# guy3540/Acoustic_Locating_VQ-VAE

Hardware: AMD Instinct MI355X
Metric: spectrograms/sec (train step), speech VQ-VAE default config (higher is better)
Workload: dtype x3mx_hb

## Files before the change

acoustic_locating_vq-vae_amd/csrc/alvq_common.h:

```cpp
#pragma once
#include <hip/hip_runtime.h>
#include <stdint.h>
#include <stdio.h>

#include "../../include/alvq.h"

namespace alvq {

void set_error(const char* fmt, ...);

enum Option { OPT_WIDE_MIN_TILES, OPT_FX_ROWS, OPT_FX_NARROW, OPT_FX_EPI, OPT_CONV_V2, OPT_CONV_K3, OPT_WGRAD_V3, OPT_VQ_REG, OPT_PHAT_LDS, OPT_COUNT };
long option(int id);

inline int check_launch(const char* what) {
  hipError_t e = hipGetLastError();
  if (e != hipSuccess) {
    set_error("%s: %s", what, hipGetErrorString(e));
    return (int)e;
  }
  return ALVQ_OK;
}

#define ALVQ_REQUIRE(cond, code, ...)  \
  do {                                 \
    if (!(cond)) {                     \
      alvq::set_error(__VA_ARGS__);    \
      return (code);                   \
    }                                  \
  } while (0)

struct DeviceOnce {
  bool done[64] = {};
  bool need() {
    int d = 0;
    if (hipGetDevice(&d) != hipSuccess || d < 0 || d >= 64) return true;
    if (done[d]) return false;
    done[d] = true;
    return true;
  }
};

constexpr int kWave = 64;
constexpr int kNumXcd = 8;

// ... 19 lines not shown
```

acoustic_locating_vq-vae_amd/csrc/api.hip:

```cpp
#include <stdarg.h>
#include <stdlib.h>
#include <string.h>

#include <atomic>

#include "alvq_common.h"

namespace alvq {
static thread_local char g_err[512] = "";
void set_error(const char* fmt, ...) {
  va_list ap;
  va_start(ap, fmt);
  vsnprintf(g_err, sizeof(g_err), fmt, ap);
  va_end(ap);
}

struct OptionSpec { const char* name; const char* env; long def; };
static const OptionSpec kSpecs[OPT_COUNT] = {
    {"wide_min_tiles", "ALVQ_WIDE_MIN_TILES", 192},
    {"fx_rows", "ALVQ_FX_ROWS", 0},
    {"fx_narrow", "ALVQ_FX_NARROW", 1},
    {"fx_epi", "ALVQ_FX_EPI", 1},
    {"conv_v2", "ALVQ_CONV_V2", 1},
    {"conv_k3", "ALVQ_CONV_K3", 1},
    {"wgrad_v3", "ALVQ_WGRAD_V3", 3},
    {"vq_reg", "ALVQ_VQ_REG", 1},
    {"phat_lds", "ALVQ_PHAT_LDS", 1},
};
static std::atomic<long> g_opt[OPT_COUNT];
static std::atomic<int> g_opt_ready{0};
static void options_init() {
  if (g_opt_ready.load(std::memory_order_acquire)) return;
  for (int i = 0; i < OPT_COUNT; ++i) {
    const char* e = getenv(kSpecs[i].env);
    g_opt[i].store(e ? atol(e) : kSpecs[i].def, std::memory_order_relaxed);
  }
  g_opt_ready.store(1, std::memory_order_release);
}
long option(int id) {
  options_init();
  return g_opt[id].load(std::memory_order_relaxed);
}
}

extern "C" const char* alvq_version(void) { return "alvq 0.4.0 (gfx950)"; }
extern "C" const char* alvq_last_error(void) { return alvq::g_err; }

extern "C" int alvq_set_option(const char* name, int64_t value) {
  ALVQ_REQUIRE(name, ALVQ_EINVAL, "alvq_set_option: null name");
  alvq::options_init();
  for (int i = 0; i < alvq::OPT_COUNT; ++i)
    if (!strcmp(name, alvq::kSpecs[i].name)) {
      alvq::g_opt[i].store((long)value, std::memory_order_relaxed);
      return ALVQ_OK;
    }
// ... 14 lines not shown
```

acoustic_locating_vq-vae_amd/csrc/conv1d_bf16.hip:

```cpp
#include <stdlib.h>

#include "alvq_common.h"
#include "bf16_common.h"
#include "conv_tile.h"
#include "nlc_host.h"

namespace alvq {

template <int KW, int OUT, int F16 = 0>
__global__ __launch_bounds__(256, 2) void conv1d_bf16_kernel(ConvBArgs a) {
  constexpr int PAD = (KW - 1) / 2;
  extern __shared__ __attribute__((aligned(16))) unsigned char lds[];
  unsigned char* const Xb = lds;
  unsigned char* const Wb = lds + 2 * XBYTES;

  const int tid = threadIdx.x, lane = tid & 63;
  const int wave = __builtin_amdgcn_readfirstlane(tid >> 6);
  const int li = lane & 15, kq = lane >> 4;
  const int wm0 = (wave >> 1) * 64, wn0 = (wave & 1) * 64;

  const ConvTileOrigin o = conv_tile_origin<TB_M, TB_R>(a);
  const int m0 = o.m0, r0 = o.r0;
  const int Cp = a.Cp;

// ... 45 lines not shown
    }
    const unsigned char* Wc = Wb + (step & 1) * WBYTES;
    const unsigned char* Xc = Xb + (chunk & 1) * XBYTES;
#pragma unroll
    for (int s = 0; s < 2; ++s) {
      bf16x8_t af[4], bfr[4];
#pragma unroll
      for (int mi = 0; mi < 4; ++mi) {
        const int row = wm0 + mi * 16 + li;
        af[mi] = *(const bf16x8_t*)(Wc + row * 128 + (((s * 4 + kq) ^ (row & 7)) << 4));
      }
#pragma unroll
      for (int ni = 0; ni < 4; ++ni) {
        const int row = wn0 + ni * 16 + li + tap;
        bfr[ni] = *(const bf16x8_t*)(Xc + row * 128 + (((s * 4 + kq) ^ (row & 7)) << 4));
      }
#pragma unroll
      for (int mi = 0; mi < 4; ++mi)
#pragma unroll
        for (int ni = 0; ni < 4; ++ni)
          acc[mi][ni] = elem_mfma16<F16>(af[mi], bfr[ni], acc[mi][ni]);
    }
    asm volatile("s_waitcnt vmcnt(0)" ::: "memory");
    __syncthreads();
    tap = ntap;
    chunk = nchunk;
  }

  if (OUT == 0) {
    wave_epilogue_bf16<4, 4, F16>(a, acc, m0, r0, li, kq, wm0, wn0);
    return;
  }
  const float oscale = a.out_scale ? *a.out_scale : 1.f;
  float* Cs = (float*)lds;
#pragma unroll
  for (int mi = 0; mi < 4; ++mi)
#pragma unroll
    for (int ni = 0; ni < 4; ++ni) {
      const int rl = wn0 + ni * 16 + li, ml = wm0 + mi * 16 + kq * 4;
      *(f32x4*)(Cs + rl * CS + ml) = acc[mi][ni];
    }
  __syncthreads();

  const int Lp1 = a.L + 1, ndata = a.B * Lp1;
  {
    const int rl = tid & 127, row = r0 + rl;
    int b, l;
    const bool ok = row_valid(row, Lp1, ndata, &b, &l);
    if (ok) {
      for (int ml = tid >> 7; ml < TB_M; ml += 2) {
        const int m = m0 + ml;
        if (m >= a.M) break;
        a.y_ncl[((long)b * a.M + m) * a.L + l] = (Cs[rl * CS + ml] + (a.bias ? a.bias[m] : 0.f)) * oscale;
      }
    }
  }
}

template <int F16 = 0>
__global__ __launch_bounds__(256) void ncl_to_nlc_kernel(const float* x, u16* y, int B, int C, int L, int Cp, int rows_total,
                                                         const float* scale = nullptr) {
  __shared__ float tile[32][33];
  elem_saturate<F16>();
  const float sc = scale ? *scale : 1.f;
  const int ct = Cp / 32, rt = (rows_total + 31) / 32;
  const int r0 = (blockIdx.x / ct) * 32, c0 = (blockIdx.x % ct) * 32;
  (void)rt;
  const int tx = threadIdx.x & 31, ty = threadIdx.x >> 5;
  const int Lp1 = L + 1, ndata = B * Lp1;
#pragma unroll
  for (int i = 0; i < 4; ++i) {
    const int c = c0 + ty + 8 * i, row = r0 + tx;
    int b, l;
    const bool ok = row_valid(row, Lp1, ndata, &b, &l) && c < C;
    tile[ty + 8 * i][tx] = ok ? x[((long)b * C + c) * L + l] * sc : 0.f;
  }
  __syncthreads();
#pragma unroll
  for (int i = 0; i < 4; ++i) {
    const int row = r0 + ty + 8 * i, c = c0 + tx;
    if (row < rows_total) y[(long)row * Cp + c] = F16 ? (u16)(elem_pk<1>(tile[tx][ty + 8 * i], 0.f) & 0xffffu) : f2bf(tile[tx][ty + 8 * i]);
  }
}

template <int F16 = 0>
__global__ __launch_bounds__(256) void nlc_to_ncl_kernel(const u16* x, float* y, int B, int C, int L, int Cp, int rows_total,
                                                         const float* scale = nullptr) {
  __shared__ float tile[32][33];
  const float sc = scale ? *scale : 1.f;
// ... 190 lines not shown
```

acoustic_locating_vq-vae_amd/csrc/conv1d_bf16x3.hip:

```cpp
#include <stdlib.h>

#include "alvq_common.h"
#include "bf16_common.h"
#include "conv_tile.h"
#include "nlc_host.h"
#include "wgrad_bias_reduce.h"
#include "wgrad_reduce.h"
#include "wgrad_tile.h"

namespace alvq {

struct ConvX3Args {
  ConvBArgs b;
  long x_plane, wp_plane, y_plane;
};

__device__ __forceinline__ void split2(float v, u16& hi, u16& lo) {
  hi = f2bf(v);
  lo = f2bf(v - bf2f(hi));
}

__device__ __forceinline__ void split_pack8(const float (&v)[8], u32x4& hi, u32x4& lo) {
#pragma unroll
  for (int e = 0; e < 4; ++e) {
    hi[e] = f2bf_pk(v[2 * e], v[2 * e + 1]);
    lo[e] = f2bf_pk(v[2 * e] - __uint_as_float(hi[e] << 16), v[2 * e + 1] - __uint_as_float(hi[e] & 0xffff0000u));
  }
}

template <int NNI>
__device__ __forceinline__ void wave_epilogue_x3(const ConvX3Args& ax, const f32x4 (&acc)[8][NNI], int m0, int r0, int li,
                                                 int kq, int wm0, int wn0) {
  const ConvBArgs& a = ax.b;
  const int Lp1 = a.L + 1, ndata = a.B * Lp1;
  const int mb0 = m0 + wm0 + (kq & 1) * 16 + (kq >> 1) * 8;
  const long pl = ax.y_plane;
#pragma unroll
  for (int ni = 0; ni < NNI; ++ni) {
    const int row = r0 + wn0 + ni * 16 + li;
    int b, l;
    const bool ok = row_valid(row, Lp1, ndata, &b, &l);
    const bool gaps = !__all(ok);
    const long o0 = (long)row * a.Mop + mb0;
    u16x8 s1h[4], s1l[4], mk[4];
#pragma unroll
    for (int mp = 0; mp < 8; mp += 2) {
      if (m0 + wm0 + mp * 16 >= a.Mop) continue;
// ... 55 lines not shown
          hi[e] = ok ? hi[e] : 0u;
          lo[e] = ok ? lo[e] : 0u;
        }
      }
      *(u32x4*)(a.y + o) = hi;
      *(u32x4*)(a.y + pl + o) = lo;
      if (a.y2) {
        const u16x8 ph = *(const u16x8*)(a.post + o), pq = *(const u16x8*)(a.post + pl + o);
#pragma unroll
        for (int e = 0; e < 8; ++e) v[e] += bf2f(ph[e]) + bf2f(pq[e]);
        split_pack8(v, hi, lo);
        if (gaps) {
#pragma unroll
          for (int e = 0; e < 4; ++e) {
            hi[e] = ok ? hi[e] : 0u;
            lo[e] = ok ? lo[e] : 0u;
          }
        }
        *(u32x4*)(a.y2 + o) = hi;
        *(u32x4*)(a.y2 + pl + o) = lo;
      }
    }
  }
}

template <int NNI, int OPS>
__device__ __forceinline__ void wave_epilogue_x3_ordered(const ConvX3Args& ax, f32x4 (&acc)[8][NNI], int m0, int r0, int li,
                                                         int kq, int wm0, int wn0) {
  const ConvBArgs& a = ax.b;
  const int Lp1 = a.L + 1, ndata = a.B * Lp1;
  const int mb0 = m0 + wm0 + (kq & 1) * 16 + (kq >> 1) * 8;
  const long pl = ax.y_plane;
  const long o00 = (long)(r0 + wn0 + li) * a.Mop + mb0, oblk = (long)16 * a.Mop;
  u16x8 s1h[4], s1l[4];
  auto request = [&](int ni) {
#pragma unroll
    for (int p = 0; p < 4; ++p) {
      s1h[p] = *(const u16x8*)(a.skip1 + o00 + ni * oblk + p * 32);
      s1l[p] = *(const u16x8*)(a.skip1 + pl + o00 + ni * oblk + p * 32);
    }
  };
  if (OPS == 1) request(0);
  if (OPS == 2) {
#pragma unroll
    for (int mi = 0; mi < 8; ++mi) {
      const int c0 = m0 + wm0 + mi * 16 + kq * 4;
      f32x4 bv;
      if (m0 + wm0 + (mi & ~1) * 16 + 32 <= a.M) {
        bv = *(const f32x4*)(a.bias + c0);
      } else {
#pragma unroll
        for (int e = 0; e < 4; ++e) bv[e] = (c0 + e < a.M) ? a.bias[c0 + e] : 0.f;
      }
#pragma unroll
      for (int ni = 0; ni < NNI; ++ni)
#pragma unroll
        for (int e = 0; e < 4; ++e) acc[mi][ni][e] += bv[e];
    }
  }
  __builtin_amdgcn_sched_barrier(0);
#pragma unroll
  for (int ni = 0; ni < NNI; ++ni) {
    int b, l;
    const bool ok = row_valid(r0 + wn0 + ni * 16 + li, Lp1, ndata, &b, &l);
    const bool gaps = !__all(ok);
    u32x4 hi[4], lo[4];
#pragma unroll
    for (int p = 0; p < 4; ++p) {
      float v[8];
#pragma unroll
      for (int e = 0; e < 4; ++e) {
        const u32x2 r = __builtin_amdgcn_permlane16_swap(__float_as_uint(acc[2 * p][ni][e]), __float_as_uint(acc[2 * p + 1][ni][e]),
                                                         false, false);
        v[e] = __uint_as_float(r[0]);
        v[e + 4] = __uint_as_float(r[1]);
      }
      if (OPS == 1) {
#pragma unroll
        for (int e = 0; e < 8; ++e) v[e] += bf2f(s1h[p][e]) + bf2f(s1l[p][e]);
      }
      if (a.relu & 1) {
#pragma unroll
        for (int e = 0; e < 8; ++e) v[e] = fmaxf(v[e], 0.f);
      }
      split_pack8(v, hi[p], lo[p]);
      if (gaps) {
#pragma unroll
        for (int e = 0; e < 4; ++e) {
          hi[p][e] = ok ? hi[p][e] : 0u;
          lo[p][e] = ok ? lo[p][e] : 0u;
        }
      }
    }
    __builtin_amdgcn_sched_barrier(0);
    if (OPS == 1 && ni + 1 < NNI) request(ni + 1);
    __builtin_amdgcn_sched_barrier(0);
#pragma unroll
    for (int p = 0; p < 4; ++p) {
      *(u32x4*)(a.y + o00 + ni * oblk + p * 32) = hi[p];
      *(u32x4*)(a.y + pl + o00 + ni * oblk + p * 32) = lo[p];
    }
  }
}


template <int OUT, int KW, int NNI = 4>
__global__ __launch_bounds__(512, 2) void conv1d_bf16x3_kernel(ConvX3Args ax) {
  static_assert(NNI == 4 || NNI == 2 || NNI == 1, "4, 2 or 1 row fragments per wave");
  typedef ConvRings G;
  constexpr int MT = NNI == 4 ? G::M : 128;
  constexpr int RT = NNI == 1 ? 128 : G::R;
  const ConvBArgs& a = ax.b;
  extern __shared__ __attribute__((aligned(16))) unsigned char lds[];
  const int tid = threadIdx.x, lane = tid & 63;
  const int wave = __builtin_amdgcn_readfirstlane(tid >> 6);
  const int li = lane & 15, kq = lane >> 4;
  const int wm0 = NNI == 4 ? (wave >> 2) * 128 : 0, wn0 = NNI == 4 ? (wave & 3) * 64 : wave * 16 * NNI;

  const ConvTileOrigin o = conv_tile_origin<MT, RT>(a);
  const int m0 = o.m0, r0 = o.r0;
  const int Cp = a.Cp;
  const int srow = slab64_lane(lane).row;
  const unsigned lane_off = slab64_lane_off(lane, Cp);
  const long tap_w = (long)a.Mp128 * Cp * 2;
  const long row16 = (long)Cp * 32;
  const long wpl = ax.wp_plane * 2, xpl = ax.x_plane * 2;
  const char* const wb = (const char*)(a.wp + ((long)m0 + wave * 32) * Cp);
  const char* const xb = (const char*)(a.x + ((long)r0 - (KW - 1) / 2 + wave * 32) * Cp);
  const ConvRingStager<KW, MT, RT, false> st(wave, srow, lane_off, tap_w, row16, wpl, xpl, wb, xb);

  const int loffA = slab64_frag16(li, kq, 0);
  int loffB[KW];
#pragma unroll
// ... 38 lines not shown
  X3_MM(fa0, BY, 0) X3_SB X3_RDA(fa1, 1, WS, 1) X3_SB                                              \
  X3_MM(fa0, BY, 1) X3_SB                                                                          \
  asm volatile("s_waitcnt vmcnt(0) lgkmcnt(0)" ::: "memory");                                      \
  __builtin_amdgcn_s_barrier();                                                                    \
  if (early) { DMA_ }                                                                              \
  X3_MM(fa1, BX, 0) X3_SB X3_RDA(fa0, 0, NWS, 0) X3_RDB(BY, NXS, NTAP, 0) X3_SB                    \
  if (!early) { DMA_ }                                                                             \
  X3_MM(fa1, BX, 1) X3_SB X3_RDA(fa0, 1, NWS, 0) X3_SB

  if (KW == 3) {
    for (int c = 0; c < nch; c += 2) {
      const int t = 3 * c;
      X3_TILE(0, 0, 0, 1, 0, 1, fb0, fb1, if (t + 2 < n) st.issueW(lds, t + 2); if (c + 1 < nch) st.issueX(lds, c + 1, 0);)
      X3_TILE(1, 0, 1, 0, 0, 2, fb1, fb0, if (t + 3 < n) st.issueW(lds, t + 3); if (c + 1 < nch) st.issueX(lds, c + 1, 1);)
      X3_TILE(0, 0, 2, 1, 1, 0, fb0, fb1, if (t + 4 < n) st.issueW(lds, t + 4);)
      X3_TILE(1, 1, 0, 0, 1, 1, fb1, fb0, if (t + 5 < n) st.issueW(lds, t + 5); if (c + 2 < nch) st.issueX(lds, c + 2, 0);)
      X3_TILE(0, 1, 1, 1, 1, 2, fb0, fb1, if (t + 6 < n) st.issueW(lds, t + 6); if (c + 2 < nch) st.issueX(lds, c + 2, 1);)
      X3_TILE(1, 1, 2, 0, 0, 0, fb1, fb0, if (t + 7 < n) st.issueW(lds, t + 7);)
    }
  } else {
    for (int t = 0; t < n; t += 2) {
      X3_TILE(0, 0, 0, 1, 1, 0, fb0, fb1, if (t + 2 < n) { st.issueW(lds, t + 2); st.issueX(lds, t + 2, 0); st.issueX(lds, t + 2, 1); })
      X3_TILE(1, 1, 0, 0, 0, 0, fb1, fb0, if (t + 3 < n) { st.issueW(lds, t + 3); st.issueX(lds, t + 3, 0); st.issueX(lds, t + 3, 1); })
    }
  }
#undef X3_TILE
#undef X3_SB
#undef X3_MM
#undef X3_RDB
#undef X3_RDA
  asm volatile("s_nop 15\n\ts_nop 15" ::: "memory");

  if constexpr (OUT == 0) {
    const bool plain = !a.skip2 && !a.mask && !a.y2 && m0 + wm0 + 128 <= a.Mop;
    if (plain && a.skip1 && !a.bias) wave_epilogue_x3_ordered<NNI, 1>(ax, acc, m0, r0, li, kq, wm0, wn0);
    else if (plain && a.bias && !a.skip1) wave_epilogue_x3_ordered<NNI, 2>(ax, acc, m0, r0, li, kq, wm0, wn0);
    else wave_epilogue_x3(ax, acc, m0, r0, li, kq, wm0, wn0);
    return;
  }
  __syncthreads();
  conv_store_ncl<false, MT, RT>(a, lds, m0, r0, tid, nullptr, [&](float* Cs, int slab) {
    if ((wn0 >> 6) == slab) store_frags16<C_SLAB_STRIDE>(Cs, acc, li, kq, wm0, wn0 & 63);
  });
}

struct WgradX3Args {
  const u16* dy[WGRAD_MAXSEG];
  const u16* x[WGRAD_MAXSEG];
  int nseg;
  float* partial;
  float* bias_partial;
  long dy_plane, x_plane;
  int Mp, Cp, M, C;
  int mtiles, ctiles, splits, chunks_per_split, total_rows;
};

template <int KW, int NCF>
__global__ __launch_bounds__(512, 2) void conv1d_wgrad_bf16x3_kernel(WgradX3Args a) {
  constexpr int MT = 128, CT = 4 * NCF * 16;
  typedef WgradSlabs<KW, MT, CT, 2> Slabs;
  constexpr int YRB = Slabs::YRB, XRB = Slabs::XRB, YBYTES = Slabs::YBYTES, XBYTES = Slabs::XBYTES;
  extern __shared__ __attribute__((aligned(16))) unsigned char lds[];

  const int tid = threadIdx.x, lane = tid & 63;
  const int wave = __builtin_amdgcn_readfirstlane(tid >> 6);
  const int wm0 = (wave >> 2) * 64, wc0 = (wave & 3) * NCF * 16;
  const WgradWork w = wgrad_work<MT, CT>(a);
  const int n = w.n;
  WgradStager<WgradX3Args, KW, MT, CT, 2, LdsDmaAsm> st(a, wave, lane, w);

  int ybase, xbase[KW], yseg[4], xseg[NCF], xline[NCF];
  wgrad_frag16_bases<KW, NCF, YRB, XRB>(lane, wm0, wc0, ybase, xbase, yseg, xseg, xline);
// ... 183 lines not shown
}

extern "C" int alvq_relu_mask_bf16x3(const void* dy, const void* t, void* out, int B, int C, int L, void* stream) {
  if (int rc = check_nlc_dims("alvq_relu_mask_bf16x3", dy && t && out, B, C, L)) return rc;
  const NlcDims d(B, C, L);
  const long n = (long)d.rows * d.Cp;
  long g = (n / 8 + 1023) / 1024;
  if (g > 2048) g = 2048;
  hipLaunchKernelGGL(relu_mask_x3_kernel, dim3((int)g), dim3(256), 0, (hipStream_t)stream, (const u16*)dy, (const u16*)t,
                     (u16*)out, d.plane / 8, n / 8);
  return check_launch("alvq_relu_mask_bf16x3");
}

static constexpr int x3_slot(int OUT, int KW, int NNI) { return ((NNI >> 1) * 2 + OUT) * 2 + (KW == 3); }
typedef KernelTable<void (*)(ConvX3Args), 12> X3Table;
static X3Table x3_table() {
  X3Table t;
  for_values<1, 2, 4>([&](auto nni) { for_values<0, 1>([&](auto out) { for_values<1, 3>([&](auto kw) {
    t.put(x3_slot(out, kw, nni), conv1d_bf16x3_kernel<out, kw, nni>, ConvRings::LDS);
  }); }); });
  return t;
}

extern "C" int alvq_conv1d_bf16x3(const void* x, const void* wp, const float* bias, const void* skip1, const void* skip2,
                                  const void* mask, const void* post, void* y, void* y2, float* y_ncl, int B, int C, int M,
                                  int L, int KW, int relu, void* stream) {
  if (int rc = check_conv_args("alvq_conv1d_bf16x3", x, wp, skip1, skip2, mask, post, y, y2, y_ncl, B, C, M, L, KW, relu, nullptr,
                               nullptr))
    return rc;
  const long rows = alvq_nlc_rows(B, L);
  ConvX3Args a{{(const u16*)x, (const u16*)wp, bias, (const u16*)skip1, (const u16*)skip2, (const u16*)mask, (const u16*)post,
                (u16*)y, (u16*)y2, y_ncl, B, L, pad_to(C, 64), M, pad_to(M, 64), pad_to(M, WP_ROWS), relu ? 1 : 0,
                (int)(rows / ConvRings::R), pad_to(M, ConvRings::M) / ConvRings::M},
               nlc_plane_elems(B, L, C), (long)alvq_packed_weight_elems(M, C, KW), nlc_plane_elems(B, L, M)};
  static const X3Table table = x3_table();
  static DeviceOnce attr;
  if (attr.need()) table.raise_lds_limit();
  const int forced = (int)option(OPT_FX_ROWS);
  const bool narrow = option(OPT_FX_NARROW) != 0 && (M <= 128 || (forced != 256 && a.b.rtiles * a.b.mtiles < 192) || forced == 128);
  if (narrow) a.b.mtiles = pad_to(M, 128) / 128;
  const bool small = narrow && forced != 256 && (a.b.rtiles * a.b.mtiles < 192 || forced == 128);
  if (small) a.b.rtiles = (int)(rows / 128);
  return table.launch(x3_slot(y ? 0 : 1, KW, small ? 1 : narrow ? 2 : 4), dim3(a.b.rtiles * a.b.mtiles), dim3(512),
                      (hipStream_t)stream, "alvq_conv1d_bf16x3", a);
}

extern "C" int64_t alvq_conv1d_wgrad_bf16x3_workspace_bytes(int B, int C, int M, int L, int KW) {
  return wgrad_workspace_bytes(B, C, M, L, KW, wgrad_x3_tile(KW), X3_BIAS_SPLITS);
}

extern "C" int alvq_conv1d_wgrad_bf16x3_splits(int B, int C, int M, int L, int KW, int nseg) {
  return wgrad_splits(B, C, M, L, KW, nseg, wgrad_x3_tile(KW));
}

static int wgrad_x3(const char* who, const void* const* dy, const void* const* x, int nseg, bool multi, float* dw, float* dbias,
                    void* workspace, int B, int C, int M, int L, int KW, int w_layout, int accumulate, hipStream_t s) {
  if (int rc = check_wgrad_args(who, dy, x, nseg, multi, dw, workspace, B, C, M, L, KW, w_layout, accumulate, false)) return rc;
  WgradX3Args a{};
  float* bpart;
  if (int rc = wgrad_plan("alvq_conv1d_wgrad_bf16x3", a, dy, x, nseg, workspace, B, C, M, L, KW, wgrad_x3_tile(KW), &bpart)) return rc;
  if (dbias) a.bias_partial = bpart;
  static const auto table = [] {
    KernelTable<void (*)(WgradX3Args), 2> t;
    for_values<1, 3>([&](auto kw) {
      constexpr int NCF = kw == 3 ? 2 : 4;
      t.put(kw == 3, conv1d_wgrad_bf16x3_kernel<kw, NCF>, wgrad_x3_lds<kw, NCF>());
    });
// ... 24 lines not shown
```

acoustic_locating_vq-vae_amd/csrc/conv1d_f16mx.hip:

```cpp
#include <stdlib.h>

#include "alvq_common.h"
#include "conv_tile.h"
#include "f16mx_common.h"
#include "nlc_host.h"

namespace alvq {

struct ConvFxArgs {
  ConvBArgs b;
  long x_plane, wp_plane, y_plane;
  int ea, eb;
  const float* out_scale;
  int* range_flag;
  unsigned long long* stamps;
  int dbg;
};

__device__ __forceinline__ void fx_join16(const u32x4& h0, const u32x4& h1, const u32x4& ql, float s_lo, float (&v)[16]) {
#pragma unroll
  for (int e = 0; e < 4; ++e) {
    float a0, a1, b0, b1;
    fx_join2(h0[e], ql[e >> 1], (e & 1) * 2, s_lo, a0, a1);
    fx_join2(h1[e], ql[2 + (e >> 1)], (e & 1) * 2, s_lo, b0, b1);
// ... 395 lines not shown
    }
  }
#undef FX_TILE
#undef FX_DMA_L
#undef FX_DMA_E
#undef FX_RD
#undef FX_SB
#undef FX_Q
#undef FX_H
#undef FX_RDQ_B
#undef FX_RDQ_A
#undef FX_RDQ
#undef FX_RDH_B
#undef FX_RDH_A
  asm volatile("s_nop 15\n\ts_nop 15" ::: "memory");

  if (DBG) st2 = __builtin_amdgcn_s_memrealtime();
  if (dbg & 8) {
    if (acc[0][0][0] == 12345.678f) a.y[0] = 1;
    return;
  }
  if (OUT == 0) {
    if constexpr (EPI != 0) wave_epilogue_fx_set<NIN, EPI>(ax, acc, m0, r0, lane, wm0, wn0);
    else wave_epilogue_fx<NIN, DBG>(ax, acc, m0, r0, lane, wm0, wn0);
    if (DBG && (dbg & (256 | 512))) {
      asm volatile("s_waitcnt vmcnt(0)" ::: "memory");
      __syncthreads();
      if (tid == 0) {
        unsigned long long* o = ax.stamps + (long)blockIdx.x * 4;
        o[0] = st0; o[1] = st1; o[2] = st2; o[3] = __builtin_amdgcn_s_memrealtime();
      }
    }
    return;
  }
  __syncthreads();
  conv_store_ncl<true, MT, RT>(a, lds, m0, r0, tid, ax.out_scale, [&](float* Cs, int slab) {
    if ((wn0 >> 6) != slab) return;
#pragma unroll
    for (int mi = 0; mi < MIN; ++mi)
#pragma unroll
      for (int ni = 0; ni < NIN; ++ni)
#pragma unroll
        for (int q4 = 0; q4 < 4; ++q4) {
          const int rl = (wn0 & 63) + ni * 32 + r32, ml = wm0 + mi * 32 + 8 * q4 + 4 * g;
          *(f32x4*)(Cs + rl * C_SLAB_STRIDE + ml) =
              f32x4{acc[mi][ni][4 * q4], acc[mi][ni][4 * q4 + 1], acc[mi][ni][4 * q4 + 2], acc[mi][ni][4 * q4 + 3]};
        }
  });
}

__device__ int g_fx_range_flag = 0;
__device__ int g_fx_range_sticky = 0;

int* fx_range_flag_ptr() {
  static int* cache[64] = {};
  int d = 0;
  if (hipGetDevice(&d) != hipSuccess || d < 0 || d >= 64) d = 0;
  if (!cache[d]) {
    void* p = nullptr;
    if (hipGetSymbolAddress(&p, HIP_SYMBOL(g_fx_range_flag)) == hipSuccess) cache[d] = (int*)p;
  }
  return cache[d];
}

int* fx_range_sticky_ptr() {
  static int* cache[64] = {};
// ... 293 lines not shown
```

acoustic_locating_vq-vae_amd/csrc/conv_tile.h:

```cpp
#pragma once
#include "alvq_common.h"
#include "bf16_common.h"

namespace alvq {

struct ConvTileOrigin {
  int m0, r0;
};
template <int MT, int RT>
__device__ __forceinline__ ConvTileOrigin conv_tile_origin(const ConvBArgs& a) {
  const int tile = xcd_remap(blockIdx.x, a.mtiles * a.rtiles);
  return {(tile % a.mtiles) * MT, (tile / a.mtiles) * RT};
}

enum SlabKey { SLAB_KEY_ROWS, SLAB_KEY_TAPS };
template <SlabKey KEY = SLAB_KEY_ROWS>
__device__ __forceinline__ int slab64_key(int quad) {
  return KEY == SLAB_KEY_TAPS ? (quad & 1) * 2 : (quad == 0 ? 0 : 4 - quad);
}

struct Slab64Lane {
  int row, grp;
};
template <SlabKey KEY = SLAB_KEY_ROWS>
// ... 83 lines not shown
  }
  __device__ __forceinline__ void prologue(unsigned char* lds, int n, int nch) const {
    issueX(lds, 0, 0);
    issueX(lds, 0, 1);
    issueW(lds, 0);
    if (n > 1) issueW(lds, 1);
    if (KW == 1 && nch > 1) {
      issueX(lds, 1, 0);
      issueX(lds, 1, 1);
    }
    asm volatile("s_waitcnt vmcnt(0)" ::: "memory");
    __builtin_amdgcn_s_barrier();
  }
 private:
  template <bool GUARDED>
  __device__ __forceinline__ void pieceW_(unsigned char* lds, int t, int k) const {
    if constexpr (GUARDED)
      if (wave * 32 >= MT) return;
    const int chunk = t / KW, tap = t - chunk * KW;
    const unsigned dst = lds_addr(lds) + (t & 1) * G::WSTAGE + wave * 2048 + (k >> 1) * G::SLAB + (k & 1) * 1024;
    lds_dma16(wb + tap * tap_w + chunk * (G::K * 2) + (k >> 1) * wpl + (k & 1) * row16, dst, lane_off);
  }
  template <bool GUARDED>
  __device__ __forceinline__ void pieceX_(unsigned char* lds, int chunk, int plane, int k) const {
    const unsigned dst = lds_addr(lds) + G::XBASE + (chunk & 1) * G::XSTAGE + plane * G::XSLAB + wave * 2048;
    const char* xs = xb + plane * xpl + chunk * (G::K * 2);
    if constexpr (GUARDED)
      if (wave * 32 >= RT) return;
    if (k < 2) lds_dma16(xs + k * row16, dst + k * 1024, lane_off);
    else if (KW == 3 && wave == RT / 32 - 1 && srow < 2) lds_dma16(xs + 2 * row16, dst + 2048, lane_off);
  }
};

template <bool SCALED, int MT, int RT, class Write>
__device__ __forceinline__ void conv_store_ncl(const ConvBArgs& a, unsigned char* lds, int m0, int r0, int tid,
                                               const float* out_scale, Write write) {
  float oscale = 1.f;
  if constexpr (SCALED) oscale = out_scale ? *out_scale : 1.f;
  float* Cs = (float*)lds;
  for (int slab = 0; slab < RT / 64; ++slab) {
    write(Cs, slab);
    __syncthreads();
    const int Lp1 = a.L + 1, ndata = a.B * Lp1;
    const int rl = tid & 63, row = r0 + slab * 64 + rl;
    int b, l;
    if (row_valid(row, Lp1, ndata, &b, &l)) {
      for (int ml = tid >> 6; ml < MT; ml += 8) {
        const int m = m0 + ml;
        if (m >= a.M) break;
        const float v = Cs[rl * C_SLAB_STRIDE + ml] + (a.bias ? a.bias[m] : 0.f);
        a.y_ncl[((long)b * a.M + m) * a.L + l] = SCALED ? v * oscale : v;
      }
    }
    __syncthreads();
  }
}

template <int CSTRIDE, int NMI, int NNI>
__device__ __forceinline__ void store_frags16(float* Cs, const f32x4 (&acc)[NMI][NNI], int li, int kq, int wm0, int rl0) {
#pragma unroll
  for (int mi = 0; mi < NMI; ++mi)
#pragma unroll
    for (int ni = 0; ni < NNI; ++ni) {
      const int rl = rl0 + ni * 16 + li, ml = wm0 + mi * 16 + kq * 4;
      *(f32x4*)(Cs + rl * CSTRIDE + ml) = acc[mi][ni];
    }
}

struct FragSet {
  bf16x8_t a[8];
  bf16x8_t b[4];
};

template <int NMI, int NNI, int F16 = 0>
__device__ __forceinline__ void wave_epilogue_bf16(const ConvBArgs& a, const f32x4 (&acc)[NMI][NNI], int m0, int r0, int li,
                                                   int kq, int wm0, int wn0);

template <int NMI, int NNI, int F16, bool S1, bool S2, bool BITS>
__device__ __forceinline__ void wave_epilogue_dgrad16(const ConvBArgs& a, const f32x4 (&acc)[NMI][NNI], int m0, int r0, int li,
                                                      int kq, int wm0, int wn0);

template <int OUT, int F16 = 0>
__device__ __forceinline__ void tile256_epilogue(const ConvBArgs& a, const f32x4 (&acc)[8][4], unsigned char* lds, int m0,
                                                 int r0, int wave, int tid, int li, int kq, int wm0) {
  if (OUT == 0) {
    const int wn0 = (wave & 3) * 64;
    const bool dgrad = (a.mask_bits || a.mask) && !a.bias && !a.y2 && !a.bits_out && !(a.relu & 1) && (a.skip1 || !a.skip2) &&
                       m0 + wm0 + 128 <= a.Mop;
    if (!dgrad) wave_epilogue_bf16<8, 4, F16>(a, acc, m0, r0, li, kq, wm0, wn0);
    else if (a.mask_bits) {
      if (a.skip2) wave_epilogue_dgrad16<8, 4, F16, true, true, true>(a, acc, m0, r0, li, kq, wm0, wn0);
      else if (a.skip1) wave_epilogue_dgrad16<8, 4, F16, true, false, true>(a, acc, m0, r0, li, kq, wm0, wn0);
      else wave_epilogue_dgrad16<8, 4, F16, false, false, true>(a, acc, m0, r0, li, kq, wm0, wn0);
    } else {
      if (a.skip2) wave_epilogue_dgrad16<8, 4, F16, true, true, false>(a, acc, m0, r0, li, kq, wm0, wn0);
      else if (a.skip1) wave_epilogue_dgrad16<8, 4, F16, true, false, false>(a, acc, m0, r0, li, kq, wm0, wn0);
      else wave_epilogue_dgrad16<8, 4, F16, false, false, false>(a, acc, m0, r0, li, kq, wm0, wn0);
    }
    return;
  }
  conv_store_ncl<true, V2_M, V2_R>(a, lds, m0, r0, tid, a.out_scale, [&](float* Cs, int slab) {
    if ((wave & 3) == slab) store_frags16<C_SLAB_STRIDE>(Cs, acc, li, kq, wm0, 0);
  });
}

template <int NMI, int NNI, int F16>
__device__ __forceinline__ void wave_epilogue_bf16(const ConvBArgs& a, const f32x4 (&acc)[NMI][NNI], int m0, int r0, int li,
                                                   int kq, int wm0, int wn0) {
  static_assert(NMI % 2 == 0, "fragments are swapped in pairs");
  elem_saturate<F16>();
  unsigned watch = 0;
  const int Lp1 = a.L + 1, ndata = a.B * Lp1;
  const int mb0 = m0 + wm0 + (kq & 1) * 16 + (kq >> 1) * 8;
#pragma unroll
  for (int ni = 0; ni < NNI; ++ni) {
    const int row = r0 + wn0 + ni * 16 + li;
    int b, l;
    const bool ok = row_valid(row, Lp1, ndata, &b, &l);
    const bool gaps = !__all(ok);
    const long o0 = (long)row * a.Mop + mb0;
    u16x8 s1[NMI / 2], s2[NMI / 2], mk[NMI / 2];
#pragma unroll
    for (int mp = 0; mp < NMI; mp += 2) {
      if (m0 + wm0 + mp * 16 >= a.Mop) continue;
      if (a.skip1) s1[mp / 2] = *(const u16x8*)(a.skip1 + o0 + mp * 16);
      if (a.skip2) s2[mp / 2] = *(const u16x8*)(a.skip2 + o0 + mp * 16);
      if (a.mask && !a.mask_bits) mk[mp / 2] = *(const u16x8*)(a.mask + o0 + mp * 16);
    }
    __builtin_amdgcn_sched_barrier(0);
#pragma unroll
    for (int mp = 0; mp < NMI; mp += 2) {
      if (m0 + wm0 + mp * 16 >= a.Mop) continue;
      const long o = o0 + mp * 16;
// ... 170 lines not shown
```

acoustic_locating_vq-vae_amd/src/acoustic_locating_vq_vae/_native.py:

```python
from __future__ import annotations

import collections
import ctypes
import functools
import os

import torch

_LIB = None
_HERE = os.path.dirname(os.path.abspath(__file__))
_DEFAULT_LIB = os.path.normpath(os.path.join(_HERE, "..", "..", "lib", "libalvq.so"))

W_OIK = 0
W_IOK = 1
VQ_PARTIALS = 1024
EW_PARTIALS = 1024

_c_void_p = ctypes.c_void_p
_i32 = ctypes.c_int
_i64 = ctypes.c_int64
_f32 = ctypes.c_float

_SIGNATURES = {
    "alvq_version": (ctypes.c_char_p, []),
# ... 1513 lines not shown
def adam_segments(param, grad, exp_avg, exp_avg_sq, segments, scalars, beta1=0.9, beta2=0.999, eps=1e-8, skip=None):
    segments = [(int(a), int(b)) for a, b in segments if b > a]
    if not segments:
        return
    lo = (ctypes.c_int64 * len(segments))(*[a for a, _ in segments])
    hi = (ctypes.c_int64 * len(segments))(*[b for _, b in segments])
    _check(lib().alvq_adam_segments_f32(_ptr(param, name="param"), _ptr(grad, name="grad"), _ptr(exp_avg, name="exp_avg"),
                                        _ptr(exp_avg_sq, name="exp_avg_sq"), lo, hi, len(segments), _ptr(scalars, name="scalars"),
                                        float(beta1), float(beta2), float(eps), _ptr(skip, name="skip"), _stream()),
           "alvq_adam_segments_f32")


def relu_mask_bf16(dy, t):
    f = _FORMATS[dy.fmt]
    out = nlc_like(dy, dy.C)
    dims = (dy.rows * dy.Cp,) if f.relu_flat else (dy.B, dy.C, dy.L)
    _check(getattr(lib(), f.relu)(dy.ptr, _nlc_ptr(t, dy, dy.C, "t"), out.ptr, *dims, _stream()), f.relu)
    return out


USE_SIGN_BITS = os.environ.get("ALVQ_SIGN_BITS", "1") != "0"


def conv1d_bf16(x, packed, bias=None, skip1=None, skip2=None, mask=None, post=None, relu=False, out_ncl=False):
    f = _FORMATS[x.fmt]
    wp, (M, C, KW, wcode) = packed
    if C != x.C:
        raise RuntimeError("conv1d_bf16: weight expects %d input channels, x has %d" % (C, x.C))
    if wcode not in f.wreads:
        raise RuntimeError("conv1d_bf16: weight packed for format %d, activation is %s" % (wcode, x.fmt))
    if bias is not None and bias.numel() != M:
        raise RuntimeError("conv1d_bf16: bias has %d elements, expected %d" % (bias.numel(), M))
    y = y2 = y_ncl = None
    if out_ncl:
        y_ncl = torch.empty((x.B, M, x.L), device=wp.device, dtype=torch.float32)
    else:
        y = nlc_like(x, M)
        y2 = nlc_like(x, M) if post is not None else None
    family = f.conv_family(int(bool(out_ncl)), KW, M, x.rows)
    extra = ()
    mask_ptr = _nlc_ptr(mask, x, M, "mask")
    bits_out = f.bits and y is not None and relu and USE_SIGN_BITS
    if f.bits:
        mask_bits = None
        if mask is not None and mask.has_bits and USE_SIGN_BITS:
            mask_bits, mask_ptr = mask.bits_ptr, None
        extra = (mask_bits, y.bits_ptr if bits_out else None)
    if f.scaled:
        extra += (_sptr(x.gscale, 1) if out_ncl else None,)
    with _timed(family, 2.0 * x.B * x.L * M * C * KW):
        rc = getattr(lib(), f.conv)(x.ptr, wp.data_ptr(), _ptr(bias, name="bias"), _nlc_ptr(skip1, x, M, "skip1"),
                                    _nlc_ptr(skip2, x, M, "skip2"), mask_ptr, _nlc_ptr(post, x, M, "post"),
                                    y.ptr if y is not None else None, y2.ptr if y2 is not None else None, _ptr(y_ncl),
                                    x.B, C, M, x.L, KW, int(bool(relu)), *extra, _stream())
    if bits_out:
        y.has_bits = True
    _check(rc, f.conv)
    if out_ncl:
        return y_ncl
    return (y, y2) if post is not None else y


def _wgrad_out(who, dy, x, KW, w_layout, dw_out, accumulate):
    shape = (dy.C, x.C, KW) if w_layout == W_OIK else (x.C, dy.C, KW)
    if dw_out is None:
        return torch.empty(shape, device=x.storage.device, dtype=torch.float32), False
    if tuple(dw_out.shape) != shape:
# ... 138 lines not shown
```

Before: 7946.

## Fold bias into accumulators, batch NCL column stores, add fused skip+post x3 epilogue

Adds the bias to the MFMA accumulator fragments before they are staged to LDS, so the NCL store loops no longer read bias per element. The NCL store is rewritten so each wave writes a strided column in batched groups instead of a per-element loop with a bounds break. A new ordered x3 epilogue variant (OPS=3) writes both the skip-added output and the post-added second output in a single pass, gated by a new x3_epi option. The Python wrapper can also accept a preallocated NCL output tensor. The cost is higher register pressure in the new epilogue and more code paths to keep correct.

Result: no change. 7985 (median of 6 runs) (+0.5%).

```diff
diff --git a/acoustic_locating_vq-vae_amd/csrc/alvq_common.h b/acoustic_locating_vq-vae_amd/csrc/alvq_common.h
--- a/acoustic_locating_vq-vae_amd/csrc/alvq_common.h
+++ b/acoustic_locating_vq-vae_amd/csrc/alvq_common.h
@@ -9,7 +9,7 @@
 
 void set_error(const char* fmt, ...);
 
-enum Option { OPT_WIDE_MIN_TILES, OPT_FX_ROWS, OPT_FX_NARROW, OPT_FX_EPI, OPT_CONV_V2, OPT_CONV_K3, OPT_WGRAD_V3, OPT_VQ_REG, OPT_PHAT_LDS, OPT_COUNT };
+enum Option { OPT_WIDE_MIN_TILES, OPT_FX_ROWS, OPT_FX_NARROW, OPT_FX_EPI, OPT_X3_EPI, OPT_CONV_V2, OPT_CONV_K3, OPT_WGRAD_V3, OPT_VQ_REG, OPT_PHAT_LDS, OPT_COUNT };
 long option(int id);
 
 inline int check_launch(const char* what) {
diff --git a/acoustic_locating_vq-vae_amd/csrc/api.hip b/acoustic_locating_vq-vae_amd/csrc/api.hip
--- a/acoustic_locating_vq-vae_amd/csrc/api.hip
+++ b/acoustic_locating_vq-vae_amd/csrc/api.hip
@@ -21,6 +21,7 @@
     {"fx_rows", "ALVQ_FX_ROWS", 0},
     {"fx_narrow", "ALVQ_FX_NARROW", 1},
     {"fx_epi", "ALVQ_FX_EPI", 1},
+    {"x3_epi", "ALVQ_X3_EPI", 1},
     {"conv_v2", "ALVQ_CONV_V2", 1},
     {"conv_k3", "ALVQ_CONV_K3", 1},
     {"wgrad_v3", "ALVQ_WGRAD_V3", 3},
diff --git a/acoustic_locating_vq-vae_amd/csrc/conv1d_bf16.hip b/acoustic_locating_vq-vae_amd/csrc/conv1d_bf16.hip
--- a/acoustic_locating_vq-vae_amd/csrc/conv1d_bf16.hip
+++ b/acoustic_locating_vq-vae_amd/csrc/conv1d_bf16.hip
@@ -101,6 +101,7 @@
     return;
   }
   const float oscale = a.out_scale ? *a.out_scale : 1.f;
+  frags16_add_bias(acc, a.bias, a.M, m0 + wm0, kq);
   float* Cs = (float*)lds;
 #pragma unroll
   for (int mi = 0; mi < 4; ++mi)
@@ -112,18 +113,11 @@
   __syncthreads();
 
   const int Lp1 = a.L + 1, ndata = a.B * Lp1;
-  {
-    const int rl = tid & 127, row = r0 + rl;
-    int b, l;
-    const bool ok = row_valid(row, Lp1, ndata, &b, &l);
-    if (ok) {
-      for (int ml = tid >> 7; ml < TB_M; ml += 2) {
-        const int m = m0 + ml;
-        if (m >= a.M) break;
-        a.y_ncl[((long)b * a.M + m) * a.L + l] = (Cs[rl * CS + ml] + (a.bias ? a.bias[m] : 0.f)) * oscale;
-      }
-    }
-  }
+  const int rl = tid & 127, half = wave >> 1;
+  int b, l;
+  if (row_valid(r0 + rl, Lp1, ndata, &b, &l))
+    ncl_store_column<TB_M / 2, 2, true>(Cs + rl * CS + half, a.y_ncl + ((long)b * a.M + m0 + half) * a.L + l, a.L,
+                                        (a.M - m0 - half + 1) >> 1, oscale);
 }
 
 template <int F16 = 0>
diff --git a/acoustic_locating_vq-vae_amd/csrc/conv1d_bf16x3.hip b/acoustic_locating_vq-vae_amd/csrc/conv1d_bf16x3.hip
--- a/acoustic_locating_vq-vae_amd/csrc/conv1d_bf16x3.hip
+++ b/acoustic_locating_vq-vae_amd/csrc/conv1d_bf16x3.hip
@@ -13,6 +13,7 @@
 struct ConvX3Args {
   ConvBArgs b;
   long x_plane, wp_plane, y_plane;
+  int ordered;
 };
 
 __device__ __forceinline__ void split2(float v, u16& hi, u16& lo) {
@@ -134,15 +135,25 @@
   const int mb0 = m0 + wm0 + (kq & 1) * 16 + (kq >> 1) * 8;
   const long pl = ax.y_plane;
   const long o00 = (long)(r0 + wn0 + li) * a.Mop + mb0, oblk = (long)16 * a.Mop;
-  u16x8 s1h[4], s1l[4];
-  auto request = [&](int ni) {
-#pragma unroll
-    for (int p = 0; p < 4; ++p) {
-      s1h[p] = *(const u16x8*)(a.skip1 + o00 + ni * oblk + p * 32);
-      s1l[p] = *(const u16x8*)(a.skip1 + pl + o00 + ni * oblk + p * 32);
+  constexpr bool S1 = OPS == 1 || OPS == 3, POST = OPS == 3;
+  constexpr int PP = POST ? 2 : 4, SPB = 4 / PP;
+  u16x8 s1h[PP], s1l[PP], psh[PP], psl[PP];
+  auto request = [&](int step) {
+    const long o = o00 + (step / SPB) * oblk + (step % SPB) * PP * 32;
+#pragma unroll
+    for (int p = 0; p < PP; ++p) {
+      s1h[p] = *(const u16x8*)(a.skip1 + o + p * 32);
+      s1l[p] = *(const u16x8*)(a.skip1 + pl + o + p * 32);
+    }
+    if (POST) {
+#pragma unroll
+      for (int p = 0; p < PP; ++p) {
+        psh[p] = *(const u16x8*)(a.post + o + p * 32);
+        psl[p] = *(const u16x8*)(a.post + pl + o + p * 32);
+      }
     }
   };
-  if (OPS == 1) request(0);
+  if (S1) request(0);
   if (OPS == 2) {
 #pragma unroll
     for (int mi = 0; mi < 8; ++mi) {
@@ -162,22 +173,23 @@
   }
   __builtin_amdgcn_sched_barrier(0);
 #pragma unroll
-  for (int ni = 0; ni < NNI; ++ni) {
+  for (int step = 0; step < NNI * SPB; ++step) {
+    const int ni = step / SPB, p0 = (step % SPB) * PP;
     int b, l;
     const bool ok = row_valid(r0 + wn0 + ni * 16 + li, Lp1, ndata, &b, &l);
     const bool gaps = !__all(ok);
-    u32x4 hi[4], lo[4];
-#pragma unroll
-    for (int p = 0; p < 4; ++p) {
+    u32x4 hi[PP], lo[PP], hi2[PP], lo2[PP];
+#pragma unroll
+    for (int p = 0; p < PP; ++p) {
       float v[8];
 #pragma unroll
       for (int e = 0; e < 4; ++e) {
-        const u32x2 r = __builtin_amdgcn_permlane16_swap(__float_as_uint(acc[2 * p][ni][e]), __float_as_uint(acc[2 * p + 1][ni][e]),
-                                                         false, false);
+        const u32x2 r = __builtin_amdgcn_permlane16_swap(__float_as_uint(acc[2 * (p0 + p)][ni][e]),
+                                                         __float_as_uint(acc[2 * (p0 + p) + 1][ni][e]), false, false);
         v[e] = __uint_as_float(r[0]);
         v[e + 4] = __uint_as_float(r[1]);
       }
-      if (OPS == 1) {
+      if (S1) {
 #pragma unroll
         for (int e = 0; e < 8; ++e) v[e] += bf2f(s1h[p][e]) + bf2f(s1l[p][e]);
       }
@@ -193,14 +205,31 @@
           lo[p][e] = ok ? lo[p][e] : 0u;
         }
       }
+      if (POST) {
+#pragma unroll
+        for (int e = 0; e < 8; ++e) v[e] += bf2f(psh[p][e]) + bf2f(psl[p][e]);
+        split_pack8(v, hi2[p], lo2[p]);
+        if (gaps) {
+#pragma unroll
+          for (int e = 0; e < 4; ++e) {
+            hi2[p][e] = ok ? hi2[p][e] : 0u;
+            lo2[p][e] = ok ? lo2[p][e] : 0u;
+          }
+        }
+      }
     }
     __builtin_amdgcn_sched_barrier(0);
-    if (OPS == 1 && ni + 1 < NNI) request(ni + 1);
+    if (S1 && step + 1 < NNI * SPB) request(step + 1);
     __builtin_amdgcn_sched_barrier(0);
-#pragma unroll
-    for (int p = 0; p < 4; ++p) {
-      *(u32x4*)(a.y + o00 + ni * oblk + p * 32) = hi[p];
-      *(u32x4*)(a.y + pl + o00 + ni * oblk + p * 32) = lo[p];
+    const long o = o00 + ni * oblk + p0 * 32;
+#pragma unroll
+    for (int p = 0; p < PP; ++p) {
+      *(u32x4*)(a.y + o + p * 32) = hi[p];
+      *(u32x4*)(a.y + pl + o + p * 32) = lo[p];
+      if (POST) {
+        *(u32x4*)(a.y2 + o + p * 32) = hi2[p];
+        *(u32x4*)(a.y2 + pl + o + p * 32) = lo2[p];
+      }
     }
   }
 }
@@ -305,12 +334,14 @@
   asm volatile("s_nop 15\n\ts_nop 15" ::: "memory");
 
   if constexpr (OUT == 0) {
-    const bool plain = !a.skip2 && !a.mask && !a.y2 && m0 + wm0 + 128 <= a.Mop;
+    const bool inside = ax.ordered && !a.skip2 && !a.mask && m0 + wm0 + 128 <= a.Mop, plain = inside && !a.y2;
     if (plain && a.skip1 && !a.bias) wave_epilogue_x3_ordered<NNI, 1>(ax, acc, m0, r0, li, kq, wm0, wn0);
     else if (plain && a.bias && !a.skip1) wave_epilogue_x3_ordered<NNI, 2>(ax, acc, m0, r0, li, kq, wm0, wn0);
+    else if (inside && a.y2 && a.skip1 && !a.bias) wave_epilogue_x3_ordered<NNI, 3>(ax, acc, m0, r0, li, kq, wm0, wn0);
     else wave_epilogue_x3(ax, acc, m0, r0, li, kq, wm0, wn0);
     return;
   }
+  frags16_add_bias(acc, a.bias, a.M, m0 + wm0, kq);
   __syncthreads();
   conv_store_ncl<false, MT, RT>(a, lds, m0, r0, tid, nullptr, [&](float* Cs, int slab) {
     if ((wn0 >> 6) == slab) store_frags16<C_SLAB_STRIDE>(Cs, acc, li, kq, wm0, wn0 & 63);
@@ -560,7 +591,8 @@
   ConvX3Args a{{(const u16*)x, (const u16*)wp, bias, (const u16*)skip1, (const u16*)skip2, (const u16*)mask, (const u16*)post,
                 (u16*)y, (u16*)y2, y_ncl, B, L, pad_to(C, 64), M, pad_to(M, 64), pad_to(M, WP_ROWS), relu ? 1 : 0,
                 (int)(rows / ConvRings::R), pad_to(M, ConvRings::M) / ConvRings::M},
-               nlc_plane_elems(B, L, C), (long)alvq_packed_weight_elems(M, C, KW), nlc_plane_elems(B, L, M)};
+               nlc_plane_elems(B, L, C), (long)alvq_packed_weight_elems(M, C, KW), nlc_plane_elems(B, L, M),
+               option(OPT_X3_EPI) != 0};
   static const X3Table table = x3_table();
   static DeviceOnce attr;
   if (attr.need()) table.raise_lds_limit();
diff --git a/acoustic_locating_vq-vae_amd/csrc/conv1d_f16mx.hip b/acoustic_locating_vq-vae_amd/csrc/conv1d_f16mx.hip
--- a/acoustic_locating_vq-vae_amd/csrc/conv1d_f16mx.hip
+++ b/acoustic_locating_vq-vae_amd/csrc/conv1d_f16mx.hip
@@ -451,6 +451,25 @@
       }
     }
     return;
+  }
+  if (a.bias) {
+#pragma unroll
+    for (int mi = 0; mi < MIN; ++mi)
+#pragma unroll
+      for (int q4 = 0; q4 < 4; ++q4) {
+        const int c0 = m0 + wm0 + mi * 32 + 8 * q4 + 4 * g;
+        f32x4 bv;
+        if (m0 + wm0 + mi * 32 + 32 <= a.M) {
+          bv = *(const f32x4*)(a.bias + c0);
+        } else {
+#pragma unroll
+          for (int e = 0; e < 4; ++e) bv[e] = (c0 + e < a.M) ? a.bias[c0 + e] : 0.f;
+        }
+#pragma unroll
+        for (int ni = 0; ni < NIN; ++ni)
+#pragma unroll
+          for (int e = 0; e < 4; ++e) acc[mi][ni][4 * q4 + e] += bv[e];
+      }
   }
   __syncthreads();
   conv_store_ncl<true, MT, RT>(a, lds, m0, r0, tid, ax.out_scale, [&](float* Cs, int slab) {
diff --git a/acoustic_locating_vq-vae_amd/csrc/conv_tile.h b/acoustic_locating_vq-vae_amd/csrc/conv_tile.h
--- a/acoustic_locating_vq-vae_amd/csrc/conv_tile.h
+++ b/acoustic_locating_vq-vae_amd/csrc/conv_tile.h
@@ -139,26 +139,62 @@
   }
 };
 
+
+template <int NMI, int NNI>
+__device__ __forceinline__ void frags16_add_bias(f32x4 (&acc)[NMI][NNI], const float* bias, int M, int mw, int kq) {
+  if (!bias) return;
+#pragma unroll
+  for (int mi = 0; mi < NMI; ++mi) {
+    const int c0 = mw + mi * 16 + kq * 4;
+    f32x4 bv;
+    if (mw + mi * 16 + 16 <= M) {
+      bv = *(const f32x4*)(bias + c0);
+    } else {
+#pragma unroll
+      for (int e = 0; e < 4; ++e) bv[e] = (c0 + e < M) ? bias[c0 + e] : 0.f;
+    }
+#pragma unroll
+    for (int ni = 0; ni < NNI; ++ni)
+#pragma unroll
+      for (int e = 0; e < 4; ++e) acc[mi][ni][e] += bv[e];
+  }
+}
+
+template <int NCH, int STEP, bool SCALED>
+__device__ __forceinline__ void ncl_store_column(const float* cs, float* y, int L, int nch, float oscale) {
+  constexpr int GRP = NCH < 16 ? NCH : 16;
+  static_assert(NCH % GRP == 0, "whole groups");
+  const long ystep = (long)STEP * L;
+#pragma unroll
+  for (int k0 = 0; k0 < NCH; k0 += GRP) {
+    if (k0 >= nch) break;
+    float v[GRP];
+#pragma unroll
+    for (int k = 0; k < GRP; ++k) v[k] = cs[(k0 + k) * STEP];
+#pragma unroll
+    for (int k = 0; k < GRP; ++k) {
+      if (k0 + k < nch) *y = SCALED ? v[k] * oscale : v[k];
+      y += ystep;
+    }
+  }
+}
+
 template <bool SCALED, int MT, int RT, class Write>
 __device__ __forceinline__ void conv_store_ncl(const ConvBArgs& a, unsigned char* lds, int m0, int r0, int tid,
                                                const float* out_scale, Write write) {
   float oscale = 1.f;
   if constexpr (SCALED) oscale = out_scale ? *out_scale : 1.f;
   float* Cs = (float*)lds;
+  const int Lp1 = a.L + 1, ndata = a.B * Lp1;
+  const int wave = __builtin_amdgcn_readfirstlane(tid >> 6), rl = tid & 63;
+  const int nch = (a.M - m0 - wave + 7) >> 3;
   for (int slab = 0; slab < RT / 64; ++slab) {
     write(Cs, slab);
     __syncthreads();
-    const int Lp1 = a.L + 1, ndata = a.B * Lp1;
-    const int rl = tid & 63, row = r0 + slab * 64 + rl;
     int b, l;
-    if (row_valid(row, Lp1, ndata, &b, &l)) {
-      for (int ml = tid >> 6; ml < MT; ml += 8) {
-        const int m = m0 + ml;
-        if (m >= a.M) break;
-        const float v = Cs[rl * C_SLAB_STRIDE + ml] + (a.bias ? a.bias[m] : 0.f);
-        a.y_ncl[((long)b * a.M + m) * a.L + l] = SCALED ? v * oscale : v;
-      }
-    }
+    if (row_valid(r0 + slab * 64 + rl, Lp1, ndata, &b, &l))
+      ncl_store_column<MT / 8, 8, SCALED>(Cs + rl * C_SLAB_STRIDE + wave, a.y_ncl + ((long)b * a.M + m0 + wave) * a.L + l, a.L, nch,
+                                          oscale);
     __syncthreads();
   }
 }
@@ -188,7 +224,7 @@
                                                       int kq, int wm0, int wn0);
 
 template <int OUT, int F16 = 0>
-__device__ __forceinline__ void tile256_epilogue(const ConvBArgs& a, const f32x4 (&acc)[8][4], unsigned char* lds, int m0,
+__device__ __forceinline__ void tile256_epilogue(const ConvBArgs& a, f32x4 (&acc)[8][4], unsigned char* lds, int m0,
                                                  int r0, int wave, int tid, int li, int kq, int wm0) {
   if (OUT == 0) {
     const int wn0 = (wave & 3) * 64;
@@ -206,6 +242,7 @@
     }
     return;
   }
+  frags16_add_bias(acc, a.bias, a.M, m0 + wm0, kq);
   conv_store_ncl<true, V2_M, V2_R>(a, lds, m0, r0, tid, a.out_scale, [&](float* Cs, int slab) {
     if ((wave & 3) == slab) store_frags16<C_SLAB_STRIDE>(Cs, acc, li, kq, wm0, 0);
   });
diff --git a/acoustic_locating_vq-vae_amd/src/acoustic_locating_vq_vae/_native.py b/acoustic_locating_vq-vae_amd/src/acoustic_locating_vq_vae/_native.py
--- a/acoustic_locating_vq-vae_amd/src/acoustic_locating_vq_vae/_native.py
+++ b/acoustic_locating_vq-vae_amd/src/acoustic_locating_vq_vae/_native.py
@@ -1569,7 +1569,11 @@
     if bias is not None and bias.numel() != M:
         raise RuntimeError("conv1d_bf16: bias has %d elements, expected %d" % (bias.numel(), M))
     y = y2 = y_ncl = None
-    if out_ncl:
+    if torch.is_tensor(out_ncl):
+        if tuple(out_ncl.shape) != (x.B, M, x.L):
+            raise RuntimeError("conv1d_bf16: out_ncl has shape %s, expected %s" % (tuple(out_ncl.shape), (x.B, M, x.L)))
+        y_ncl, out_ncl = out_ncl, True
+    elif out_ncl:
         y_ncl = torch.empty((x.B, M, x.L), device=wp.device, dtype=torch.float32)
     else:
         y = nlc_like(x, M)
```
